# VatsalSy/gerris-fft-particles

Measured on AMD Instinct MI355X. Metric: Mcell-steps/s (projection+advection), 3D 256^3 uniform, higher is better.
Workload: dtype f64; 1 GPU; 3-D periodic Taylor-Green, 256^3 per GPU, default projection/advection parameters (SURVEY 8d config C); relax_mode=exact, parallelism=1 box, rccl_world_size=0

## Files before the change

gerris-fft-particles_amd/csrc/domain.hip:

```cpp
#include "gfship_internal.hpp"

namespace gfship {

static thread_local char g_error[1024] = "";

void set_error (const char * fmt, ...)
{
  va_list ap;
  va_start (ap, fmt);
  vsnprintf (g_error, sizeof (g_error), fmt, ap);
  va_end (ap);
}

int hip_fail (hipError_t e, const char * what, const char * file, int line)
{
  set_error ("HIP error %d (%s) in %s at %s:%d", (int) e, hipGetErrorString (e), what, file, line);
  return e == hipErrorOutOfMemory ? GFSHIP_ENOMEM : GFSHIP_EHIP;
}

Field * get_field (gfship_domain * dom, gfship_field f)
{
  if (!dom || f < 0 || (size_t) f >= dom->fields.size () || !dom->fields[f].used) {
    set_error ("invalid field handle %d", f);
    return nullptr;
// ... 132 lines not shown
  return GFSHIP_OK;
}

int gfship_domain_set_exchange (gfship_domain * dom, gfship_exchange_fn fn, void * ctx)
{
  GFSHIP_CHECK (dom != nullptr, GFSHIP_EINVAL, "null domain");
  dom->exchange = fn;
  dom->exchange_ctx = ctx;
  return GFSHIP_OK;
}

int gfship_domain_set_reduce (gfship_domain * dom, gfship_reduce_fn fn, void * ctx)
{
  GFSHIP_CHECK (dom != nullptr, GFSHIP_EINVAL, "null domain");
  dom->reduce = fn;
  dom->reduce_ctx = ctx;
  return GFSHIP_OK;
}

int gfship_domain_set_gather (gfship_domain * dom, gfship_gather_fn fn, void * ctx, int rank,
			      int nboxes, const int lattice[3])
{
  GFSHIP_CHECK (dom && lattice, GFSHIP_EINVAL, "null argument");
  GFSHIP_CHECK (nboxes >= 1 && rank >= 0 && rank < nboxes &&
		(long) lattice[0]*lattice[1]*lattice[2] == nboxes, GFSHIP_EINVAL,
		"box %d of %d on a lattice of %d x %d x %d", rank, nboxes, lattice[0], lattice[1], lattice[2]);
  for (int d = 0; d < 2*dom->dim; d++)
    GFSHIP_CHECK (lattice[d/2] == 1 || dom->side[d] == GFSHIP_SIDE_EXTERNAL, GFSHIP_EINVAL,
		  "side %d faces another box of the lattice: it must be GFSHIP_SIDE_EXTERNAL", d);
  dom->gather = fn;
  dom->gather_ctx = ctx;
  dom->lat_rank = rank; dom->lat_n = nboxes;
  for (int c = 0; c < 3; c++) dom->lat_b[c] = lattice[c];
  return GFSHIP_OK;
}

int gfship_domain_path_counts (gfship_domain * dom, unsigned long long * lattice_cycles,
			       unsigned long long * fused_mpi_launches)
{
  GFSHIP_CHECK (dom != nullptr, GFSHIP_EINVAL, "null domain");
  if (lattice_cycles) *lattice_cycles = dom->n_lattice_cycles;
  if (fused_mpi_launches) *fused_mpi_launches = dom->n_fused_mpi;
  return GFSHIP_OK;
}

int gfship_domain_kernel_counts (gfship_domain * dom, unsigned long long * counts, int n)
{
  GFSHIP_CHECK (dom != nullptr && counts != nullptr && n >= 0, GFSHIP_EINVAL, "null argument");
  for (int k = 0; k < n && k < GFSHIP_KC_COUNT; k++)
    counts[k] = dom->kc[k];
  return GFSHIP_OK;
}

int gfship_domain_synchronize (gfship_domain * dom)
{
  GFSHIP_CHECK (dom != nullptr, GFSHIP_EINVAL, "null domain");
  GFSHIP_HIP (hipStreamSynchronize (dom->stream));
  return GFSHIP_OK;
}

void * gfship_domain_stream (gfship_domain * dom)
{
  return dom ? (void *) dom->stream : nullptr;
}

gfship_field gfship_field_alloc (gfship_domain * dom, int component)
{
  GFSHIP_CHECK (dom != nullptr, GFSHIP_EINVAL, "null domain");
  GFSHIP_CHECK (component >= -1 && component < dom->dim, GFSHIP_EINVAL,
		"component %d out of range", component);
  size_t slot = dom->fields.size ();
  for (size_t f = 0; f < dom->fields.size (); f++)
    if (!dom->fields[f].used) { slot = f; break; }
  if (slot == dom->fields.size ())
    dom->fields.emplace_back ();
  Field nf;
  nf.used = true;
  nf.component = component;
  size_t total = 0;
  for (int l = 0; l <= dom->depth; l++)
    total += (dom->lay[l].total + 31) & ~(size_t) 31;
  double * base = nullptr;
  GFSHIP_HIP (hipMalloc ((void **) &base, total*sizeof (double)));
  GFSHIP_HIP (hipMemsetAsync (base, 0, total*sizeof (double), dom->stream));
  size_t o = 0;
  for (int l = dom->depth; l >= 0; l--) {
    nf.lev[l] = base + o;
    nf.zero[l] = true;
    o += (dom->lay[l].total + 31) & ~(size_t) 31;
  }
  dom->fields[slot] = nf;
  return (gfship_field) slot;
}

int gfship_field_free (gfship_domain * dom, gfship_field f)
{
  Field * F = get_field (dom, f);
  if (!F) return GFSHIP_EINVAL;
  GFSHIP_HIP (hipStreamSynchronize (dom->stream));
  GFSHIP_HIP (hipFree (F->lev[dom->depth]));
  for (int d = 0; d < 6; d++)
    if (F->bcval[d]) GFSHIP_HIP (hipFree (F->bcval[d]));
  *F = Field ();
  return GFSHIP_OK;
}

// ... 131 lines not shown
```

gerris-fft-particles_amd/csrc/gfship_internal.hpp:

```cpp
#pragma once

#include <hip/hip_runtime.h>
#include <cstdio>
#include <cstdarg>
#include <cstring>
#include <vector>
#include <deque>
#include <string>
#include <type_traits>
#include "gfship.h"
#include "switches.hpp"
#include "cell_update.hpp"

namespace gfship {

struct Layout {
  int n = 0;
  int px = 0;
  int xo = 1;
  int rows = 0;
  int dim = 3;
  long sy = 0;
  long sz = 0;
  size_t total = 0;
// ... 38 lines not shown
struct RelaxOp {
  int kind = 0;
  double w = 1., h2 = 1.;
  const double * wf[6] = {};
};

inline W6 op_weights (const RelaxOp * op)
{
  W6 wf;
  for (int d = 0; d < 6; d++) wf.p[d] = op ? op->wf[d] : nullptr;
  return wf;
}

struct BcDesc {
  int side[6];
  int type[6];
  const double * val[6];
  int component;
  int homogeneous;
};

}

struct gfship_domain {
  int dim = 3, depth = 0, device = 0;
  int side[6] = {1, 1, 1, 1, 1, 1};
  int relax_mode = GFSHIP_RELAX_EXACT;
  gfship::Switches sw;
  gfship::Layout lay[GFSHIP_MAXLEVEL + 1];
  std::deque<gfship::Field> fields;
  hipStream_t stream = nullptr;
  hipEvent_t ev0 = nullptr, ev1 = nullptr;
  hipStream_t side_stream = nullptr;
  hipEvent_t side_fork = nullptr;
  int (* before_write) (void *) = nullptr;
  void * before_write_ctx = nullptr;
  double * d_scratch = nullptr;
  size_t scratch_doubles = 0;
  double * h_pinned = nullptr;
  gfship_exchange_fn exchange = nullptr; void * exchange_ctx = nullptr;
  gfship_reduce_fn reduce = nullptr;     void * reduce_ctx = nullptr;
  bool has_external = false;
  void * comm = nullptr;
  int overlap = 0;
  int lat_rank = -1, lat_n = 0, lat_b[3] = { 1, 1, 1 };
  gfship_gather_fn gather = nullptr; void * gather_ctx = nullptr;
  double * lat_res = nullptr, * lat_xch = nullptr;
  unsigned * lat_bar = nullptr;
  size_t lat_res_doubles = 0, lat_xch_doubles = 0;
  double * gfv_send[6] = {}, * gfv_recv[6] = {};
  double src[3] = { 0., 0., 0. };
  unsigned long long n_lattice_cycles = 0, n_fused_mpi = 0;
  unsigned long long kc[GFSHIP_KC_COUNT] = {};
  bool lattice_attr_set = false;
  void * mpi_plan[GFSHIP_MAXLEVEL + 1] = {};
  gfship_field dp_cache = -1;
  int skew_resident = -1;
  int patch_resident = 0;
  bool no_fused_godunov = false;
  bool no_fused_loop = false;
  bool force_hyperplane = false;
  bool unit_weights = false;
  bool weighted = false;
  unsigned long weights_stamp = 0;
  gfship_field wf[6] = {-1, -1, -1, -1, -1, -1};
  gfship::SkewPlan skew[GFSHIP_MAXLEVEL + 1];
  double diff_w[GFSHIP_MAXLEVEL + 1] = {};
  double * cfl_partial = nullptr;
  size_t cfl_nblocks = 0, cfl_used = 0;
  bool cfl_dirty = false;
  bool coarse_attr_set = false;
  gfship_field res_cache = -1;
  bool diff_ready = false;
  int diff_kind = 1;
  int patch_call = -1;
};

namespace gfship {

void set_error (const char * fmt, ...);
int  hip_fail (hipError_t e, const char * what, const char * file, int line);

inline int before_write (gfship_domain * dom)
{
  return dom->before_write ? dom->before_write (dom->before_write_ctx) : GFSHIP_OK;
}

#define GFSHIP_HIP(call) do { hipError_t e_ = (call); \
    if (e_ != hipSuccess) return gfship::hip_fail (e_, #call, __FILE__, __LINE__); } while (0)

inline hipError_t stream_wait_spin (hipStream_t st)
{
  hipError_t e;
  while ((e = hipStreamQuery (st)) == hipErrorNotReady)
    ;
  return e;
}

template <class F> inline void with_bools (F && f) { f (); }
template <class F, class... B> inline void with_bools (F && f, bool b0, B... rest)
{
  if (b0) with_bools ([&] (auto... r) { f (std::true_type {}, r...); }, rest...);
  else    with_bools ([&] (auto... r) { f (std::false_type {}, r...); }, rest...);
}

template <class F, class... B> inline void with_kind (F && f, int kind, B... bools)
// ... 182 lines not shown
```

gerris-fft-particles_amd/csrc/poisson_kernels.hip:

```cpp
#include "gfship_internal.hpp"
#include "cell_loop.hpp"
#include "relax_skew.hpp"
#include <algorithm>
#include <cstdlib>

namespace gfship {

template <int DIM, int OP>
__device__ __forceinline__ double relax_value (const double * __restrict__ u, long c, long sy, long sz,
					       double rhs, double dia, unsigned dimension,
					       double omega, double w, double h2, const W6 * wf = nullptr)
{
  return cell_update<DIM, OP> (kind_weights<OP> (w, ArrayW { wf, c }), ArrayU { u, c, sy, sz }, rhs, dia, u + c,
			       dimension, omega, h2);
}

__device__ __forceinline__ double relax_value_six (const double * __restrict__ u, long c, long sy, long sz,
						    double rhs)
{
  return cell_update_six (ArrayU { u, c, sy, sz }, rhs);
}

template <int DIM, int OP>
__global__ void __launch_bounds__(256)
// ... 1003 lines not shown
  return GFSHIP_OK;
}

template <int DIM>
__global__ void __launch_bounds__(256)
relax_redblack_kernel (Layout L, int colour, unsigned dimension, double omega,
		       double * __restrict__ u, const double * __restrict__ rhs,
		       const double * __restrict__ dia)
{
  int n = L.n;
  int half = (n + 1)/2;
  int ih = blockIdx.x*blockDim.x + threadIdx.x;
  int j = blockIdx.y + 1;
  int k = DIM == 3 ? blockIdx.z + 1 : 0;
  if (ih >= half) return;
  int i = 2*ih + 1 + ((j + k + colour) & 1);
  if (i > n) return;
  long c = L.idx (i, j, k);
  u[c] = relax_value<DIM, 0> (u, c, L.sy, L.sz, rhs[c], dia[c], dimension, omega, 1., 1.);
}

int launch_relax_redblack (gfship_domain * dom, unsigned dimension, int level, double omega,
			   double * u, const double * rhs, const double * dia)
{
  const Layout & L = dom->lay[level];
  int half = (L.n + 1)/2;
  int block = half >= 128 ? 128 : 64;
  dim3 grid ((half + block - 1)/block, L.n, dom->dim == 3 ? L.n : 1);
  for (int colour = 0; colour < 2; colour++) {
    with_bools ([&] (auto D3) {
      hipLaunchKernelGGL (relax_redblack_kernel<decltype (D3)::value ? 3 : 2>, grid, dim3 (block), 0, dom->stream,
			  L, colour, dimension, omega, u, rhs, dia);
    }, dom->dim == 3);
  }
  GFSHIP_HIP (hipGetLastError ());
  return GFSHIP_OK;
}

template <int DIM>
__global__ void __launch_bounds__(256)
residual_kernel (Layout L, const double * __restrict__ u, const double * __restrict__ rhs,
		 const double * __restrict__ dia, double * __restrict__ res)
{
  CELL_LOOP_PROLOGUE (L);
  const FaceSums s = face_sums<DIM> (UnitW {}, ArrayU { u, c, L.sy, L.sz }, dia[c]);
  res[c] = residual_close (s.a, s.b, rhs[c], u[c]);
}

template <bool NORM>
__global__ void residual_norm2_kernel (Layout L, const double * __restrict__ u, const double * __restrict__ rhs,
				       const double * __restrict__ dia, double * __restrict__ res, double inv,
				       double weight, double * __restrict__ partial);

int launch_residual (gfship_domain * dom, int level, const double * u, const double * rhs,
		     const double * dia, double * res)
{
  const Layout & L = dom->lay[level];
  dim3 grid, block;
  cell_grid (L, &grid, &block);
  const bool pairs = dom->sw.residual_pairs;
  if (dom->dim == 3 && L.n >= 64) dom->kc[pairs ? GFSHIP_KC_RESIDUAL_PAIRS : GFSHIP_KC_RESIDUAL_SCALAR]++;
  if (dom->dim == 3 && L.n >= 64 && pairs) {
    const long nitems = (long) L.n*L.n*(L.n/2);
    long nb = (nitems + 255)/256;
    if (nb > 4096) nb = 4096;
    hipLaunchKernelGGL (residual_norm2_kernel<false>, dim3 ((int) nb), dim3 (256), 0, dom->stream, L, u, rhs,
			dia, res, 1., 1., nullptr);
    GFSHIP_HIP (hipGetLastError ());
    return GFSHIP_OK;
  }
  with_bools ([&] (auto D3) {
    hipLaunchKernelGGL (residual_kernel<decltype (D3)::value ? 3 : 2>, grid, block, 0, dom->stream, L, u, rhs, dia, res);
  }, dom->dim == 3);
  GFSHIP_HIP (hipGetLastError ());
  return GFSHIP_OK;
}

template <int DIM>
__global__ void __launch_bounds__(256)
residual_weighted_kernel (Layout L, const double * __restrict__ u, const double * __restrict__ rhs,
			  const double * __restrict__ dia, double * __restrict__ res, W6 wf)
{
  CELL_LOOP_PROLOGUE (L);
  const FaceSums s = face_sums<DIM> (ArrayW { &wf, c }, ArrayU { u, c, L.sy, L.sz }, dia[c]);
  res[c] = residual_close (s.a, s.b, rhs[c], u[c]);
}

RelaxOp weighted_op (gfship_domain * dom, int level)
{
  RelaxOp op;
  op.kind = 2;
  for (int d = 0; d < 2*dom->dim; d++)
    op.wf[d] = dom->fields[dom->wf[d]].lev[level];
  return op;
}

int launch_residual_weighted (gfship_domain * dom, int level, const double * u, const double * rhs,
			      const double * dia, double * res)
{
  const Layout & L = dom->lay[level];
  dim3 grid, block;
  cell_grid (L, &grid, &block);
  RelaxOp op = weighted_op (dom, level);
  W6 wf = op_weights (&op);
  with_bools ([&] (auto D3) {
    hipLaunchKernelGGL (residual_weighted_kernel<decltype (D3)::value ? 3 : 2>, grid, block, 0, dom->stream, L, u, rhs,
			dia, res, wf);
  }, dom->dim == 3);
  GFSHIP_HIP (hipGetLastError ());
  return GFSHIP_OK;
}

struct A3 { const double * p[3]; };
struct M6 { double * p[6]; };

// ... 386 lines not shown
    if (dia) di = *(const d2 *) (dia + c);
    d2 out;
    {
      double a = di.x, b = 0.;
      a += 1.; b += 1.*uc.y;
      a += 1.; b += 1.*ul;
      a += 1.; b += 1.*ut.x;
      a += 1.; b += 1.*ub.x;
      a += 1.; b += 1.*uf.x;
      a += 1.; b += 1.*uk.x;
      out.x = rh.x - (b - uc.x*a);
    }
    {
      double a = di.y, b = 0.;
      a += 1.; b += 1.*ur;
      a += 1.; b += 1.*uc.x;
      a += 1.; b += 1.*ut.y;
      a += 1.; b += 1.*ub.y;
      a += 1.; b += 1.*uf.y;
      a += 1.; b += 1.*uk.y;
      out.y = rh.y - (b - uc.y*a);
    }
    *(d2 *) (res + c) = out;
    if (NORM)
#pragma unroll
    for (int e = 0; e < 2; e++) {
      const double raw = e ? out.y : out.x;
      double val = raw*inv;
      s0 += weight*val;
      val = fabs (val);
      s3 = fmax (s3, val);
      s1 += weight*val;
      s2 += weight*val*val;
      s4 += raw;
    }
  }
  if (!NORM) return;
  __shared__ double sh[5][4];
  s0 = wave_sum (s0); s1 = wave_sum (s1); s2 = wave_sum (s2); s3 = wave_max (s3); s4 = wave_sum (s4);
  int w = threadIdx.x >> 6, lane = threadIdx.x & 63;
  if (lane == 0) { sh[0][w] = s0; sh[1][w] = s1; sh[2][w] = s2; sh[3][w] = s3; sh[4][w] = s4; }
  __syncthreads ();
  if (threadIdx.x == 0) {
    int nw = blockDim.x >> 6;
    double r0 = 0., r1 = 0., r2 = 0., r3 = 0., r4 = 0.;
    for (int q = 0; q < nw; q++) {
      r0 += sh[0][q]; r1 += sh[1][q]; r2 += sh[2][q]; r3 = fmax (r3, sh[3][q]); r4 += sh[4][q];
    }
    double * p = partial + 5*(size_t) blockIdx.x;
    p[0] = r0; p[1] = r1; p[2] = r2; p[3] = r3; p[4] = r4;
  }
}

int launch_residual_norm (gfship_domain * dom, int level, const double * u, const double * rhs,
			  const double * dia, double * res, double scale, double weight,
			  double * out, bool dia_zero)
{
  const Layout & L = dom->lay[level];
  if (!power_of_two (scale)) {
    int r = launch_residual (dom, level, u, rhs, dia, res);
    if (r) return r;
    return out ? launch_norm (dom, level, res, scale, weight, out) :
      launch_norm_async (dom, level, res, scale, weight);
  }
  long nrows = L.dim == 3 ? (long) L.n*L.n : L.n;
  int block = L.n >= 256 ? 256 : L.n >= 128 ? 128 : 64;
  int rn_blocks = dom->sw.rn_blocks;
  if (rn_blocks < 64 || rn_blocks > 8192) rn_blocks = 4096;
  int nblocks = (int) (nrows > rn_blocks ? rn_blocks : nrows);
  double * partial = dom->d_scratch;
  double * result = out ? dom->h_pinned : dom->h_pinned + 8;
  const bool rn_pairs = dom->sw.residual_pairs;
  if (dom->dim == 3 && L.n >= 64) dom->kc[rn_pairs ? GFSHIP_KC_RESIDUAL_PAIRS : GFSHIP_KC_RESIDUAL_SCALAR]++;
  if (dom->dim == 3 && L.n >= 64 && rn_pairs) {
    const long nitems = (long) L.n*L.n*(L.n/2);
    long nb = (nitems + 255)/256;
    nblocks = (int) (nb > rn_blocks ? rn_blocks : nb);
    hipLaunchKernelGGL (residual_norm2_kernel<true>, dim3 (nblocks), dim3 (256), 0, dom->stream, L, u,
			rhs, dia_zero ? nullptr : dia, res, 1./scale, weight, partial);
  }
  else
    with_bools ([&] (auto D3) {
      hipLaunchKernelGGL (residual_norm_kernel<decltype (D3)::value ? 3 : 2>, dim3 (nblocks), dim3 (block), 0,
			  dom->stream, L, u, rhs, dia_zero ? nullptr : dia, res, 1./scale, weight, partial);
    }, dom->dim == 3);
  hipLaunchKernelGGL (norm_final_kernel, dim3 (1), dim3 (256), 0, dom->stream,
		      partial, nblocks, result);
  GFSHIP_HIP (hipGetLastError ());
  dom->kc[GFSHIP_KC_RN_BLOCKS_LIMIT] = rn_blocks;
  if ((unsigned long long) nblocks > dom->kc[GFSHIP_KC_RN_BLOCKS_MAX])
    dom->kc[GFSHIP_KC_RN_BLOCKS_MAX] = nblocks;
  if (out) {
    GFSHIP_HIP (stream_wait_spin (dom->stream));
    memcpy (out, dom->h_pinned, 5*sizeof (double));
  }
  return GFSHIP_OK;
}

struct MpiOrderPlan {
  int * cells = nullptr;
  std::vector<int> first;
  int shell_steps = 0;
};

template <int DIM, int OP>
__global__ void __launch_bounds__(256)
relax_listed_kernel (const int * __restrict__ cells, int count, long sy, long sz,
		     unsigned dimension, double omega, double w, double h2,
		     double * __restrict__ u, const double * __restrict__ rhs,
		     const double * __restrict__ dia)
{
  const int q = blockIdx.x*blockDim.x + threadIdx.x;
  if (q >= count) return;
  const long c = cells[q];
  u[c] = relax_value<DIM, OP> (u, c, sy, sz, rhs[c], dia[c], dimension, omega, w, h2);
}

static inline unsigned long long morton_key (int dim, int level, int I, int J, int K)
{
  unsigned long long m = 0;
  for (int b = level - 1; b >= 0; b--) {
    unsigned n = ((I >> b) & 1) | (((J >> b) & 1) << 1) | (dim == 3 ? ((K >> b) & 1) << 2 : 0);
    m = (m << (dim == 3 ? 3 : 2)) | n;
  }
  return m;
}

// ... 126 lines not shown
```

gerris-fft-particles_amd/gfship/__init__.py:

```python
import ctypes as C
import os
import sys

import numpy as np

_PKG = os.path.dirname(os.path.dirname(os.path.abspath(__file__)))
LIB_PATH = os.environ.get("GFSHIP_LIB", os.path.join(_PKG, "lib", "libgfship.so"))

SIDE_PERIODIC, SIDE_BOUNDARY, SIDE_EXTERNAL = 0, 1, 2
BC_SYMMETRY, BC_DIRICHLET, BC_NEUMANN = 0, 1, 2
SCHEME_GODUNOV, SCHEME_NONE = 0, 1
RELAX_EXACT, RELAX_REDBLACK, RELAX_EXACT_HYPERPLANE, RELAX_EXACT_PER_SWEEP = 0, 1, 2, 3


class GfshipError(RuntimeError):
    pass


class Norm(C.Structure):
    _fields_ = [("bias", C.c_double), ("first", C.c_double), ("second", C.c_double),
                ("infty", C.c_double), ("w", C.c_double)]


class MultilevelParams(C.Structure):
# ... 47 lines not shown
    "gfship_diffusion_rhs": (_i, [_vp, _i, _i, _i, _d]),
    "gfship_diffusion_residual": (_i, [_vp, _i, _i, _i, _i]),
    "gfship_diffusion_cycle": (_i, [_vp, _u, _u, _u, _i, _i, _i, _i]),
    "gfship_diffusion": (_i, [_vp, C.POINTER(MultilevelParams), _i, _i, _i]),
    "gfship_time_relax": (_i, [_vp, _u, _i, _i, _i, _i, _i, _pd]),
    "gfship_time_relax_loop": (_i, [_vp, _i, _i, _i, _i, _u, _i, _pd, _pi]),
    "gfship_time_relax_loop_inclusive": (_i, [_vp, _i, _i, _i, _i, _u, _i, _pd, _pi, _pd]),
    "gfship_sim_create": (_i, [C.POINTER(_vp), _vp]),
    "gfship_sim_destroy": (None, [_vp]),
    "gfship_sim_variable": (_i, [_vp, _i, _i]),
    "gfship_sim_projection_params": (C.POINTER(MultilevelParams), [_vp]),
    "gfship_sim_approx_projection_params": (C.POINTER(MultilevelParams), [_vp]),
    "gfship_sim_advection_params": (C.POINTER(AdvectionParams), [_vp]),
    "gfship_sim_set_time": (_i, [_vp, _d, _d]),
    "gfship_sim_set_next_event": (_i, [_vp, _vp, _vp]),
    "gfship_sim_time": (_d, [_vp]),
    "gfship_sim_iter": (_u, [_vp]),
    "gfship_sim_add_tracer": (_i, [_vp]),
    "gfship_sim_set_viscosity": (_i, [_vp, _i, _d]),
    "gfship_sim_set_viscosity_faces": (_i, [_vp, _i, _pi]),
    "gfship_sim_set_alpha_cell": (_i, [_vp, _i]),
    "gfship_sim_set_viscosity_cell": (_i, [_vp, _i]),
    "gfship_variable_mac_source": (_i, [_vp, _i, _i]),
    "gfship_sim_set_alpha": (_i, [_vp, _pi]),
    "gfship_sim_set_source": (_i, [_vp, _i, _d]),
    "gfship_sim_diffusion_params": (C.POINTER(MultilevelParams), [_vp, _i]),
    "gfship_sim_start": (_i, [_vp]),
    "gfship_sim_step": (_i, [_vp]),
    "gfship_sim_advection_step": (_i, [_vp]),
    "gfship_sim_set_tracer_gradient": (_i, [_vp, _i, _i]),
    "gfship_sim_set_tracer_scheme": (_i, [_vp, _i, _i]),
    "gfship_sim_set_tracer_diffusion": (_i, [_vp, _i, _d]),
    "gfship_sim_tracer_diffusion_params": (C.POINTER(MultilevelParams), [_vp, _i]),
    "gfship_sim_tracer_diffusion_path": (_i, [_vp, _i]),
    "gfship_sim_tracer_diffusion_counts": (_i, [_vp, C.POINTER(C.c_ulonglong)]),
    "gfship_predicted_face_velocities": (_i, [_vp]),
    "gfship_mac_projection": (_i, [_vp, C.POINTER(MultilevelParams), _d, _i, _pi]),
    "gfship_approximate_projection": (_i, [_vp, C.POINTER(MultilevelParams), _d, _i, _pi]),
    "gfship_centered_velocity_advection": (_i, [_vp, _pi, _pi]),
    "gfship_correct_centered_velocities": (_i, [_vp, _pi, _d]),
    "gfship_sim_advance_time": (_i, [_vp]),
    "gfship_tracer_advection": (_i, [_vp, _i, _d]),
    "gfship_domain_cfl": (_i, [_vp, _pd]),
    "gfship_set_timestep": (_i, [_vp]),
    "gfship_coarse_init": (_i, [_vp]),
    "gfship_divergence_norm": (_i, [_vp, C.POINTER(Norm)]),
    "gfship_sim_download_un": (_i, [_vp, _i, _pd]),
    "gfship_domain_set_overlap": (_i, [_vp, _i]),
    "gfship_domain_set_exchange": (_i, [_vp, _vp, _vp]),
    "gfship_domain_set_reduce": (_i, [_vp, _vp, _vp]),
    "gfship_domain_set_gather": (_i, [_vp, _vp, _vp, _i, _i, C.POINTER(C.c_int)]),
    "gfship_domain_path_counts": (_i, [_vp, C.POINTER(C.c_ulonglong), C.POINTER(C.c_ulonglong)]),
    "gfship_domain_kernel_counts": (_i, [_vp, C.POINTER(C.c_ulonglong), _i]),
    "gfship_sim_restart": (_i, [_vp, _d, _u]),
    "gfship_snapshot_tree_bytes": (C.c_size_t, [_vp, _i]),
    "gfship_snapshot_tree_write": (_i, [_vp, _i, _pi, _vp, C.c_size_t]),
    "gfship_snapshot_tree_read": (_i, [_vp, _i, _pi, _vp, C.c_size_t]),
    "gfship_comm_available": (_i, []),
    "gfship_comm_unique_id": (_i, [_vp]),
    "gfship_domain_comm_init": (_i, [_vp, _vp, _i, _i, _pi]),
    "gfship_domain_comm_size": (_i, [_vp]),
    "gfship_domain_comm_stats": (_i, [_vp, C.POINTER(C.c_ulonglong), C.POINTER(C.c_ulonglong)]),
    "gfship_domain_comm_destroy": (_i, [_vp]),
    "gfship_halo_pack": (_i, [_vp, _vp, _i, _i, _vp]),
    "gfship_halo_unpack": (_i, [_vp, _vp, _i, _i, _vp]),
    "gfship_halo_pack_sides": (_i, [_vp, _vp, _i, _i, _pi, C.POINTER(_vp)]),
    "gfship_halo_unpack_sides": (_i, [_vp, _vp, _i, _i, _pi, C.POINTER(_vp)]),
    "gfship_field_interpolate": (_i, [_vp, _i, _i, _pd, _pd, C.POINTER(C.c_ubyte)]),
    "gfship_particles_create": (_i, [C.POINTER(_vp), _vp, _i, _pd, C.POINTER(C.c_uint)]),
    "gfship_particles_destroy": (None, [_vp]),
    "gfship_particle_list_event": (_i, [_vp]),
    "gfship_particles_count": (_i, [_vp]),
    "gfship_particles_set_migrate": (_i, [_vp, _vp, _vp]),
    "gfship_particles_slots": (_i, [_vp]),
    "gfship_particles_record_size": (_i, [_vp]),
    "gfship_particles_sort": (_i, [_vp]),
    "gfship_particles_set_sort_interval": (_i, [_vp, _i]),
    "gfship_particles_download": (_i, [_vp, _pd, C.POINTER(C.c_uint)]),
    "gfship_particles_download_old": (_i, [_vp, _pd]),
    "gfship_energy_spectra_bins": (_i, [_vp]),
    "gfship_energy_spectra": (_i, [_vp, _i, C.POINTER(_i), _pd, C.POINTER(C.c_double),
                                   C.POINTER(C.c_double)]),
    "gfship_init_spectra": (_i, [_vp, _vp, C.POINTER(_i)]),
    "gfship_output_spectra_side": (_i, [_vp]),
    "gfship_output_spectra": (_i, [_vp, _i, _pd, C.POINTER(C.c_double)]),
    "gfship_output_spectra_plane": (_i, [_vp, _i, _i, _d, _pd, _pd]),
    "gfship_turbulent_viscosity": (_i, [_vp, C.POINTER(_i), C.c_double, _i, _i]),
    "gfship_particles_set_particulate": (_i, [_vp, _pd, _pd, _pd]),
    "gfship_particles_set_forces": (_i, [_vp, _i, C.POINTER(_i), _pd]),
    "gfship_particles_set_force_coefficient": (_i, [_vp, _i, C.c_char_p]),
    "gfship_particles_download_particulate": (_i, [_vp, _pd, _pd, _pd]),
    "gfship_particulate_field": (_i, [_vp, _i]),
    "gfship_particles_forces_on_fluid": (_i, [_vp]),
    "gfship_particles_set_kernel": (_i, [_vp, C.c_double, C.c_char_p]),
    "gfship_source_particulate_event": (_i, [_vp, C.POINTER(_i)]),
    "gfship_particles_spread_forces": (_i, [_vp, C.POINTER(_i)]),
    "gfship_sim_set_source_fields": (_i, [_vp, C.POINTER(_i)]),
    "gfship_particles_time_spreading": (_i, [_vp, C.POINTER(_i), _pd]),
    "gfship_tree_create": (_i, [C.POINTER(_vp), _i, C.c_void_p, _vp, _i]),
    "gfship_tree_create_sides": (_i, [C.POINTER(_vp), _i, C.c_void_p, _vp, _pi, _i]),
    "gfship_tree_set_bc": (_i, [_vp, _i, _i]),
    "gfship_tree_poisson_solve": (_i, [_vp, C.POINTER(MultilevelParams), _d]),
    "gfship_tree_destroy": (None, [_vp]),
    "gfship_tree_depth": (_i, [_vp]),
    "gfship_tree_dim": (_i, [_vp]),
    "gfship_tree_flags": (_i, [_vp, _i, C.POINTER(C.c_ubyte)]),
    "gfship_tree_upload": (_i, [_vp, _i, _i, _pd]),
    "gfship_tree_download": (_i, [_vp, _i, _i, _pd]),
    "gfship_tree_projection_params": (C.POINTER(MultilevelParams), [_vp, _i]),
    "gfship_tree_set_time": (_i, [_vp, _d, _d]),
    "gfship_tree_set_next_event": (_i, [_vp, _vp, _vp]),
    "gfship_tree_time": (_d, [_vp]),
    "gfship_tree_dt": (_d, [_vp]),
    "gfship_tree_iter": (_u, [_vp]),
    "gfship_tree_add_tracer": (_i, [_vp, _i]),
    "gfship_tree_set_bc_u": (_i, [_vp, _i, _i, _i]),
    "gfship_tree_set_viscosity": (_i, [_vp, _i, _d]),
    "gfship_tree_set_source": (_i, [_vp, _i, _d]),
    "gfship_tree_diffusion_params": (C.POINTER(MultilevelParams), [_vp, _i]),
    "gfship_tree_start": (_i, [_vp]),
    "gfship_tree_step": (_i, [_vp]),
    "gfship_tree_snapshot_bytes": (C.c_size_t, [_vp, _i]),
    "gfship_tree_snapshot_write": (_i, [_vp, _i, _pi, _vp, C.c_size_t]),
    "gfship_tree_snapshot_read": (_i, [_vp, _i, _pi, _vp, C.c_size_t]),
    "gfship_tree_restart": (_i, [_vp, _d, _u]),
    "gfship_tree_sweep_levels": (_i, [_vp, _i, _pi, _pi]),
    "gfship_tree_divergence": (_i, [_vp]),
    "gfship_tree_host_check": (_i, [_i, C.c_void_p, _vp, _pi, _u, C.POINTER(C.c_longlong)]),
    "gfship_tree_host_check_diffusion": (_i, [_i, C.c_void_p, _vp, _pi, _u, _d, C.POINTER(C.c_longlong)]),
}


UNIQUE_ID_BYTES = 128

KERNEL_COUNT_NAMES = (
    "PREDICT_SWEEP", "PREDICT_SWEEP_MPI", "PREDICT_TILED", "PREDICT_TILED_MPI", "PREDICT_GENERAL",
    "ADVECT3_SWEEP2", "ADVECT3_SWEEP2_MPI", "ADVECT3_SWEEP1", "ADVECT3_TILED", "ADVECT3_TILED_MPI",
    "ADVECT1_TILED_VELOCITY", "ADVECT1_TILED_TRACER", "ADVECT_GENERAL", "CORRECTION_FUSED",
    "CORRECTION_DECLINED", "DIVERGENCE_FUSED", "DIVERGENCE_DECLINED", "DIVERGENCE_SEPARATE",
    "PROJECT_PAIRS", "PROJECT_SCALAR", "RESIDUAL_PAIRS", "RESIDUAL_SCALAR", "RN_BLOCKS_LIMIT",
    "RN_BLOCKS_MAX", "ROWS2D", "HYPERPLANES_2D", "DIFFUSION_PIPELINED", "DIFFUSION_HYPERPLANES",
    "WEIGHTED_PIPELINED", "WEIGHTED_HYPERPLANES", "PROLONGATION_FUSED", "PROLONGATION_DECLINED",
    "RESTRICTION_FUSED", "RESTRICTION_DECLINED", "PROLONG_PACK_NEW", "PROLONG_PACK_OLD",
    "ARM_AHEAD", "ARM_AHEAD_DECLINED", "ARM_INLINE", "PATCH_LOOP_KERNEL_ARMS",
    "PATCH_LOOP_HOST_ARMS", "XCD_SCOPE_ON", "XCD_SCOPE_OFF", "XCD_NEAR_MODE", "XCD_PLACE_ON",
    "XCD_PLACE_OFF", "COARSE_CYCLES", "COARSE_THREADS", "COARSE_END_BY_LEVEL",
    "DIFFUSION_FACES_PIPELINED", "DIFFUSION_FACES_HYPERPLANES",
)
KERNEL_COUNT_VALUES = ("RN_BLOCKS_LIMIT", "RN_BLOCKS_MAX", "XCD_NEAR_MODE", "COARSE_THREADS")


def comm_available():
    _check(lib().gfship_comm_available())


def comm_unique_id():
    buf = C.create_string_buffer(UNIQUE_ID_BYTES)
    _check(lib().gfship_comm_unique_id(buf))
    return buf.raw


def lib():
    global _lib
    if _lib is None:
        if not os.path.exists(LIB_PATH):
            raise GfshipError("%s not found: run __graft_entry__.build() "
                              "(gerris-fft-particles_amd/csrc/build.sh)" % LIB_PATH)
        if "torch" not in sys.modules and os.environ.get("GFSHIP_NO_TORCH") is None:
            try:
                import torch
            except ImportError:
                pass
        L = C.CDLL(LIB_PATH)
        for name, (res, args) in SIGNATURES.items():
            f = getattr(L, name)
            f.restype, f.argtypes = res, args
        _lib = L
    return _lib


def _check(rc):
    if rc < 0:
        raise GfshipError("gfship error %d: %s" % (rc, lib().gfship_last_error().decode()))
    return rc


class Variable:

    def __init__(self, dom, component=-1):
        self.dom = dom
        self.h = _check(lib().gfship_field_alloc(dom.ptr, component))

    def _shape(self, level):
        return ((1 << level) + 2,) * self.dom.dim

    def upload(self, a, level=None):
        level = self.dom.depth if level is None else level
        a = np.ascontiguousarray(a, dtype=np.float64)
        assert a.shape == self._shape(level), (a.shape, self._shape(level))
        _check(lib().gfship_field_upload(self.dom.ptr, self.h, level, a.ctypes.data_as(_pd)))

    def download(self, level=None):
# ... 10 lines not shown
        if val is not None:
            val = np.ascontiguousarray(val, dtype=np.float64).ravel()
            p = val.ctypes.data_as(_pd)
        else:
            p = None
        _check(lib().gfship_field_set_bc(self.dom.ptr, self.h, d, kind, p))

    def free(self):
        if self.h is not None and self.dom.ptr:
            lib().gfship_field_free(self.dom.ptr, self.h)
            self.h = None


class Domain:

    def __init__(self, dim, depth, side=None, device=0):
        self.dim, self.depth = dim, depth
        s = (C.c_int * 6)(*(side if side is not None else [SIDE_BOUNDARY] * 6))
        p = _vp()
        _check(lib().gfship_domain_create(C.byref(p), dim, depth, s, device))
        self.ptr = p

    def variable(self, component=-1):
        return Variable(self, component)

    def params(self):
        par = MultilevelParams()
        lib().gfship_multilevel_params_init(C.byref(par), self.dim)
        return par

    def comm_init(self, unique_id, rank, nranks, lattice):
        buf = C.create_string_buffer(bytes(unique_id), UNIQUE_ID_BYTES)
        _check(lib().gfship_domain_comm_init(self.ptr, buf, rank, nranks, (C.c_int * 3)(*lattice)))

    def comm_size(self):
        return _check(lib().gfship_domain_comm_size(self.ptr))

    def comm_stats(self):
        m, b = C.c_ulonglong(), C.c_ulonglong()
        _check(lib().gfship_domain_comm_stats(self.ptr, C.byref(m), C.byref(b)))
        return int(m.value), int(b.value)

    def path_counts(self):
        a, b = C.c_ulonglong(), C.c_ulonglong()
        _check(lib().gfship_domain_path_counts(self.ptr, C.byref(a), C.byref(b)))
        return int(a.value), int(b.value)

    def kernel_counts(self):
        n = len(KERNEL_COUNT_NAMES)
        a = (C.c_ulonglong * n)()
        _check(lib().gfship_domain_kernel_counts(self.ptr, a, n))
        return {name: int(a[k]) for k, name in enumerate(KERNEL_COUNT_NAMES)}

    def snapshot_tree(self, variables):
        n = len(variables)
        h = (C.c_int * n)(*[v.h for v in variables])
        size = lib().gfship_snapshot_tree_bytes(self.ptr, n)
        buf = C.create_string_buffer(size)
        _check(lib().gfship_snapshot_tree_write(self.ptr, n, h, buf, size))
        return buf.raw

    def snapshot_tree_read(self, variables, data):
        n = len(variables)
        h = (C.c_int * n)(*[v.h for v in variables])
        buf = C.create_string_buffer(bytes(data), len(data))
        _check(lib().gfship_snapshot_tree_read(self.ptr, n, h, buf, len(data)))

    def set_overlap(self, overlap):
        _check(lib().gfship_domain_set_overlap(self.ptr, int(overlap)))

    def set_relax_mode(self, mode):
        _check(lib().gfship_domain_set_relax_mode(self.ptr, mode))

    def synchronize(self):
        _check(lib().gfship_domain_synchronize(self.ptr))

    def bc(self, v, v1=None, level=None):
        level = self.depth if level is None else level
        _check(lib().gfship_bc(self.ptr, v.h, (v1 or v).h, level))

    def homogeneous_bc(self, ov, v, level=None):
        level = self.depth if level is None else level
        _check(lib().gfship_homogeneous_bc(self.ptr, ov.h, v.h, level))

    def poisson_coefficients(self):
        _check(lib().gfship_poisson_coefficients(self.ptr))

    def poisson_coefficients_alpha(self, alpha):
        h = (C.c_int * 3)(*([v.h for v in alpha] + [-1] * (3 - len(alpha))))
        _check(lib().gfship_poisson_coefficients_alpha(self.ptr, h))

    def poisson_weight(self, d, level=None):
        w = C.c_int()
        _check(lib().gfship_poisson_weights(self.ptr, d, C.byref(w)))
        v = Variable.__new__(Variable)
        v.dom, v.h = self, w.value
        a = v.download(level)
        v.h = None
        return a

    def relax(self, u, rhs, dia, level=None, omega=1., d=None):
        level = self.depth if level is None else level
        _check(lib().gfship_relax(self.ptr, d or self.dim, level, omega, u.h, rhs.h, dia.h))

    def residual(self, u, rhs, dia, res, level=None, d=None):
        level = self.depth if level is None else level
# ... 560 lines not shown
```

include/gfship.h:

```cpp
#ifndef GFSHIP_H
#define GFSHIP_H

#include <stddef.h>

#ifdef __cplusplus
extern "C" {
#endif

#define GFSHIP_VERSION   1
#define GFSHIP_MAXLEVEL  12

enum { GFSHIP_OK = 0, GFSHIP_EINVAL = -1, GFSHIP_ENODEVICE = -2, GFSHIP_ENOMEM = -3,
       GFSHIP_EHIP = -4, GFSHIP_EUNSUPPORTED = -5 };

enum { GFSHIP_SIDE_PERIODIC = 0,
       GFSHIP_SIDE_BOUNDARY = 1,
       GFSHIP_SIDE_EXTERNAL = 2 };

enum { GFSHIP_BC_SYMMETRY = 0, GFSHIP_BC_DIRICHLET = 1, GFSHIP_BC_NEUMANN = 2 };

enum { GFSHIP_RELAX_EXACT = 0, GFSHIP_RELAX_REDBLACK = 1, GFSHIP_RELAX_EXACT_HYPERPLANE = 2,
       GFSHIP_RELAX_EXACT_PER_SWEEP = 3 };

typedef struct gfship_domain gfship_domain;
// ... 217 lines not shown
  GFSHIP_KC_PREDICT_SWEEP_MPI,
  GFSHIP_KC_PREDICT_TILED,
  GFSHIP_KC_PREDICT_TILED_MPI,
  GFSHIP_KC_PREDICT_GENERAL,
  GFSHIP_KC_ADVECT3_SWEEP2,
  GFSHIP_KC_ADVECT3_SWEEP2_MPI,
  GFSHIP_KC_ADVECT3_SWEEP1,
  GFSHIP_KC_ADVECT3_TILED,
  GFSHIP_KC_ADVECT3_TILED_MPI,
  GFSHIP_KC_ADVECT1_TILED_VELOCITY,
  GFSHIP_KC_ADVECT1_TILED_TRACER,
  GFSHIP_KC_ADVECT_GENERAL,
  GFSHIP_KC_CORRECTION_FUSED,
  GFSHIP_KC_CORRECTION_DECLINED,
  GFSHIP_KC_DIVERGENCE_FUSED,
  GFSHIP_KC_DIVERGENCE_DECLINED,
  GFSHIP_KC_DIVERGENCE_SEPARATE,
  GFSHIP_KC_PROJECT_PAIRS,
  GFSHIP_KC_PROJECT_SCALAR,
  GFSHIP_KC_RESIDUAL_PAIRS,
  GFSHIP_KC_RESIDUAL_SCALAR,
  GFSHIP_KC_RN_BLOCKS_LIMIT,
  GFSHIP_KC_RN_BLOCKS_MAX,
  GFSHIP_KC_ROWS2D,
  GFSHIP_KC_HYPERPLANES_2D,
  GFSHIP_KC_DIFFUSION_PIPELINED,
  GFSHIP_KC_DIFFUSION_HYPERPLANES,
  GFSHIP_KC_WEIGHTED_PIPELINED,
  GFSHIP_KC_WEIGHTED_HYPERPLANES,
  GFSHIP_KC_PROLONGATION_FUSED,
  GFSHIP_KC_PROLONGATION_DECLINED,
  GFSHIP_KC_RESTRICTION_FUSED,
  GFSHIP_KC_RESTRICTION_DECLINED,
  GFSHIP_KC_PROLONG_PACK_NEW,
  GFSHIP_KC_PROLONG_PACK_OLD,
  GFSHIP_KC_ARM_AHEAD,
  GFSHIP_KC_ARM_AHEAD_DECLINED,
  GFSHIP_KC_ARM_INLINE,
  GFSHIP_KC_PATCH_LOOP_KERNEL_ARMS,
  GFSHIP_KC_PATCH_LOOP_HOST_ARMS,
  GFSHIP_KC_XCD_SCOPE_ON,
  GFSHIP_KC_XCD_SCOPE_OFF,
  GFSHIP_KC_XCD_NEAR_MODE,
  GFSHIP_KC_XCD_PLACE_ON,
  GFSHIP_KC_XCD_PLACE_OFF,
  GFSHIP_KC_COARSE_CYCLES,
  GFSHIP_KC_COARSE_THREADS,
  GFSHIP_KC_COARSE_END_BY_LEVEL,
  GFSHIP_KC_DIFFUSION_FACES_PIPELINED,
  GFSHIP_KC_DIFFUSION_FACES_HYPERPLANES,
  GFSHIP_KC_COUNT
};
int  gfship_domain_kernel_counts (gfship_domain * dom, unsigned long long * counts, int n);
#define GFSHIP_UNIQUE_ID_BYTES 128
int  gfship_comm_available (void);
int  gfship_comm_unique_id (void * id);
int  gfship_domain_comm_init (gfship_domain * dom, const void * unique_id, int rank, int nranks,
			      const int lattice[3]);
int  gfship_domain_comm_size (gfship_domain * dom);
int  gfship_domain_comm_stats (gfship_domain * dom, unsigned long long * messages,
			       unsigned long long * bytes);
int  gfship_domain_comm_destroy (gfship_domain * dom);

int  gfship_halo_pack (gfship_domain * dom, const void * dev_ptr, int level, int side, void * dev_buf);
int  gfship_halo_unpack (gfship_domain * dom, void * dev_ptr, int level, int side, const void * dev_buf);
int  gfship_halo_pack_sides (gfship_domain * dom, const void * dev_ptr, int level, int nsides,
			     const int * sides, void * const * dev_bufs);
int  gfship_halo_unpack_sides (gfship_domain * dom, void * dev_ptr, int level, int nsides,
			       const int * sides, void * const * dev_bufs);


typedef struct gfship_tree gfship_tree;
typedef double (* gfship_refine_fn) (double x, double y, double z, void * ctx);
enum { GFSHIP_TREE_P = 0, GFSHIP_TREE_PMAC, GFSHIP_TREE_U, GFSHIP_TREE_V, GFSHIP_TREE_GX, GFSHIP_TREE_GY,
       GFSHIP_TREE_GMACX, GFSHIP_TREE_GMACY, GFSHIP_TREE_UN0, GFSHIP_TREE_UN1, GFSHIP_TREE_UN2,
       GFSHIP_TREE_UN3, GFSHIP_TREE_W, GFSHIP_TREE_GZ, GFSHIP_TREE_GMACZ, GFSHIP_TREE_UN4,
       GFSHIP_TREE_UN5, GFSHIP_TREE_DIV, GFSHIP_TREE_BCVAL, GFSHIP_TREE_RES,
       GFSHIP_TREE_T0, GFSHIP_TREE_T1, GFSHIP_TREE_BCU, GFSHIP_TREE_BCV, GFSHIP_TREE_BCW };
int  gfship_tree_create (gfship_tree ** tree, int dim, gfship_refine_fn refine, void * ctx, int device);
int  gfship_tree_create_sides (gfship_tree ** tree, int dim, gfship_refine_fn refine, void * ctx,
			       const int * side, int device);
int  gfship_tree_set_bc (gfship_tree * tree, int d, int kind);
int  gfship_tree_poisson_solve (gfship_tree * tree, gfship_multilevel_params * par, double dt);
void gfship_tree_destroy (gfship_tree * tree);
int  gfship_tree_depth (const gfship_tree * tree);
int  gfship_tree_dim (const gfship_tree * tree);
int  gfship_tree_flags (const gfship_tree * tree, int level, unsigned char * out );
int  gfship_tree_upload (gfship_tree * tree, int var, int level, const double * in );
int  gfship_tree_download (gfship_tree * tree, int var, int level, double * out);
gfship_multilevel_params * gfship_tree_projection_params (gfship_tree * tree, int approx);
int  gfship_tree_set_time (gfship_tree * tree, double end, double cfl);
int  gfship_tree_set_next_event (gfship_tree * tree, gfship_next_event_fn fn, void * ctx);
double   gfship_tree_time (const gfship_tree * tree);
double   gfship_tree_dt (const gfship_tree * tree);
unsigned gfship_tree_iter (const gfship_tree * tree);
int  gfship_tree_add_tracer (gfship_tree * tree, int gradient);
int  gfship_tree_set_bc_u (gfship_tree * tree, int c, int d, int kind);
int  gfship_tree_set_viscosity (gfship_tree * tree, int c, double nu);
int  gfship_tree_set_source (gfship_tree * tree, int c, double g);
gfship_multilevel_params * gfship_tree_diffusion_params (gfship_tree * tree, int c);
int  gfship_tree_start (gfship_tree * tree);
int  gfship_tree_step (gfship_tree * tree);
size_t gfship_tree_snapshot_bytes (const gfship_tree * tree, int nvars);
int  gfship_tree_snapshot_write (gfship_tree * tree, int nvars, const int * vars, void * host_buf, size_t bytes);
int  gfship_tree_snapshot_read (gfship_tree * tree, int nvars, const int * vars, const void * host_buf, size_t bytes);
int  gfship_tree_restart (gfship_tree * tree, double t, unsigned i);
// ... 24 lines not shown
```

Baseline: 2836 Mcell-steps/s.

## Add z-marching residual kernel with shared-memory plane reuse for large grids

```diff
diff --git a/gerris-fft-particles_amd/csrc/domain.hip b/gerris-fft-particles_amd/csrc/domain.hip
--- a/gerris-fft-particles_amd/csrc/domain.hip
+++ b/gerris-fft-particles_amd/csrc/domain.hip
@@ -208,6 +208,23 @@
   return GFSHIP_OK;
 }
 
+int gfship_domain_kernel_counts_more (gfship_domain * dom, unsigned long long * counts, int n)
+{
+  GFSHIP_CHECK (dom != nullptr && counts != nullptr && n >= 0, GFSHIP_EINVAL, "null argument");
+  for (int k = 0; k < n && k < GFSHIP_KC_MORE_COUNT; k++)
+    counts[k] = dom->kc_more[k];
+  return GFSHIP_OK;
+}
+
+int gfship_domain_set_march_min_n (gfship_domain * dom, int n)
+{
+  GFSHIP_CHECK (n >= 64 && (n & (n - 1)) == 0, GFSHIP_EINVAL,
+		"march_min_n = %d: a power of two >= 64 is expected", n);
+  GFSHIP_CHECK (dom != nullptr, GFSHIP_EINVAL, "null domain");
+  dom->march_min_n = n;
+  return GFSHIP_OK;
+}
+
 int gfship_domain_synchronize (gfship_domain * dom)
 {
   GFSHIP_CHECK (dom != nullptr, GFSHIP_EINVAL, "null domain");
diff --git a/gerris-fft-particles_amd/csrc/gfship_internal.hpp b/gerris-fft-particles_amd/csrc/gfship_internal.hpp
--- a/gerris-fft-particles_amd/csrc/gfship_internal.hpp
+++ b/gerris-fft-particles_amd/csrc/gfship_internal.hpp
@@ -114,6 +114,8 @@
   double src[3] = { 0., 0., 0. };
   unsigned long long n_lattice_cycles = 0, n_fused_mpi = 0;
   unsigned long long kc[GFSHIP_KC_COUNT] = {};
+  unsigned long long kc_more[GFSHIP_KC_MORE_COUNT] = {};
+  int march_min_n = 256;
   bool lattice_attr_set = false;
   void * mpi_plan[GFSHIP_MAXLEVEL + 1] = {};
   gfship_field dp_cache = -1;
diff --git a/gerris-fft-particles_amd/csrc/poisson_kernels.hip b/gerris-fft-particles_amd/csrc/poisson_kernels.hip
--- a/gerris-fft-particles_amd/csrc/poisson_kernels.hip
+++ b/gerris-fft-particles_amd/csrc/poisson_kernels.hip
@@ -1079,6 +1079,9 @@
 				       const double * __restrict__ dia, double * __restrict__ res, double inv,
 				       double weight, double * __restrict__ partial);
 
+static bool launch_residual_march (gfship_domain * dom, const Layout & L, const double * u, const double * rhs,
+				   const double * dia, double * res);
+
 int launch_residual (gfship_domain * dom, int level, const double * u, const double * rhs,
 		     const double * dia, double * res)
 {
@@ -1088,6 +1091,10 @@
   const bool pairs = dom->sw.residual_pairs;
   if (dom->dim == 3 && L.n >= 64) dom->kc[pairs ? GFSHIP_KC_RESIDUAL_PAIRS : GFSHIP_KC_RESIDUAL_SCALAR]++;
   if (dom->dim == 3 && L.n >= 64 && pairs) {
+    if (launch_residual_march (dom, L, u, rhs, dia, res)) {
+      GFSHIP_HIP (hipGetLastError ());
+      return GFSHIP_OK;
+    }
     const long nitems = (long) L.n*L.n*(L.n/2);
     long nb = (nitems + 255)/256;
     if (nb > 4096) nb = 4096;
@@ -1580,6 +1587,178 @@
   }
 }
 
+constexpr int MARCH_CHUNK = 32, MARCH_WIDE_N = 256;
+#define MARCH_WIDE 128, 2, 2
+#define MARCH_NARROW 32, 8, 2
+
+template <bool NORM, int PX, int RY, int RT>
+__global__ void __launch_bounds__(PX*RY)
+residual_march_kernel (Layout L, const double * __restrict__ u, const double * __restrict__ rhs,
+		       const double * __restrict__ dia, double * __restrict__ res, double inv,
+		       double weight, double * __restrict__ partial, int chunk)
+{
+  typedef double d2 __attribute__((ext_vector_type(2)));
+  constexpr int NW = PX*RY/64;
+  static_assert (PX <= 64 ? 64 % PX == 0 : PX % 64 == 0, "a row segment is a part or a multiple of a wavefront");
+  __shared__ d2 plane[2][RY*RT][PX];
+  const int n = L.n, nxs = n/(2*PX);
+  const int p = threadIdx.x % PX, r = threadIdx.x / PX;
+  const int xs = blockIdx.x % nxs, yb = blockIdx.x / nxs;
+  const int k0 = 1 + blockIdx.y*chunk, k1 = min (k0 + chunk, n + 1);
+  long c = L.idx (1 + 2*(xs*PX + p), 1 + (yb*RY + r)*RT, k0);
+  const bool lo = r == 0, hi = r == RY - 1, halo = lo || hi;
+  const bool e0 = p % 64 == 0, e1 = p % 64 == 63 || p == PX - 1;
+  const long hoff = lo ? - L.sy : RT*L.sy;
+  d2 um[RT], uc[RT], up[RT], rh[RT], di[RT];
+  double ue[RT][2];
+  d2 uh = { 0., 0. };
+#pragma unroll
+  for (int t = 0; t < RT; t++) {
+    const long ct = c + t*L.sy;
+    um[t] = *(const d2 *) (u + ct - L.sz); uc[t] = *(const d2 *) (u + ct); up[t] = *(const d2 *) (u + ct + L.sz);
+    ue[t][0] = ue[t][1] = 0.;
+    if (e0) ue[t][0] = u[ct - 1];
+    if (e1) ue[t][1] = u[ct + 2];
+    rh[t] = *(const d2 *) (rhs + ct);
+    di[t] = d2 { 0., 0. };
+    if (dia) di[t] = *(const d2 *) (dia + ct);
+    plane[0][r*RT + t][p] = uc[t];
+  }
+  if (halo) uh = *(const d2 *) (u + c + hoff);
+  __syncthreads ();
+  double s0 = 0., s1 = 0., s2 = 0., s3 = 0., s4 = 0.;
+  int buf = 0;
+  for (int k = k0; k < k1; k++, c += L.sz, buf ^= 1) {
+    d2 un[RT], rhn[RT], din[RT], uhn = { 0., 0. };
+    double uen[RT][2];
+#pragma unroll
+    for (int t = 0; t < RT; t++) {
+      un[t] = rhn[t] = din[t] = d2 { 0., 0. };
+      uen[t][0] = uen[t][1] = 0.;
+    }
+    if (k + 1 < k1) {
+#pragma unroll
+      for (int t = 0; t < RT; t++) {
+	const long ct = c + t*L.sy + L.sz;
+	un[t] = *(const d2 *) (u + ct + L.sz);
+	if (e0) uen[t][0] = u[ct - 1];
+	if (e1) uen[t][1] = u[ct + 2];
+	rhn[t] = *(const d2 *) (rhs + ct);
+	if (dia) din[t] = *(const d2 *) (dia + ct);
+      }
+      if (halo) uhn = *(const d2 *) (u + c + L.sz + hoff);
+    }
+#pragma unroll
+    for (int t = 0; t < RT; t++)
+      plane[buf ^ 1][r*RT + t][p] = up[t];
+    d2 below = uh, above = uh;
+    if (!lo) below = plane[buf][r*RT - 1][p];
+    if (!hi) above = plane[buf][r*RT + RT][p];
+#pragma unroll
+    for (int t = 0; t < RT; t++) {
+      const d2 ub = t > 0 ? uc[t > 0 ? t - 1 : 0] : below, ut = t < RT - 1 ? uc[t < RT - 1 ? t + 1 : t] : above;
+      double ul = __shfl_up (uc[t].y, 1, 64), ur = __shfl_down (uc[t].x, 1, 64);
+      if (e0) ul = ue[t][0];
+      if (e1) ur = ue[t][1];
+      d2 out;
+      {
+	double a = di[t].x, b = 0.;
+	a += 1.; b += 1.*uc[t].y;
+	a += 1.; b += 1.*ul;
+	a += 1.; b += 1.*ut.x;
+	a += 1.; b += 1.*ub.x;
+	a += 1.; b += 1.*up[t].x;
+	a += 1.; b += 1.*um[t].x;
+	out.x = rh[t].x - (b - uc[t].x*a);
+      }
+      {
+	double a = di[t].y, b = 0.;
+	a += 1.; b += 1.*ur;
+	a += 1.; b += 1.*uc[t].x;
+	a += 1.; b += 1.*ut.y;
+	a += 1.; b += 1.*ub.y;
+	a += 1.; b += 1.*up[t].y;
+	a += 1.; b += 1.*um[t].y;
+	out.y = rh[t].y - (b - uc[t].y*a);
+      }
+      *(d2 *) (res + c + t*L.sy) = out;
+      if (NORM)
+#pragma unroll
+      for (int e = 0; e < 2; e++) {
+	const double raw = e ? out.y : out.x;
+	double val = raw*inv;
+	s0 += weight*val;
+	val = fabs (val);
+	s3 = fmax (s3, val);
+	s1 += weight*val;
+	s2 += weight*val*val;
+	s4 += raw;
+      }
+    }
+    __syncthreads ();
+#pragma unroll
+    for (int t = 0; t < RT; t++) {
+      um[t] = uc[t]; uc[t] = up[t]; up[t] = un[t]; rh[t] = rhn[t]; di[t] = din[t];
+      ue[t][0] = uen[t][0]; ue[t][1] = uen[t][1];
+    }
+    uh = uhn;
+  }
+  if (NORM) {
+    static_assert (NW <= 4, "block_norm_sums reduces at most 4 wavefronts");
+    block_norm_sums (s0, s1, s2, s3, s4, partial, blockIdx.x + (size_t) gridDim.x*blockIdx.y);
+  }
+}
+
+struct MarchPlan { dim3 grid; int chunk; bool wide; };
+
+static bool march_plan (gfship_domain * dom, const Layout & L, MarchPlan * m)
+{
+  if (dom->dim != 3 || !dom->sw.residual_pairs || dom->sw.rn_blocks != 0 || L.n < dom->march_min_n || L.n % 64)
+    return false;
+  constexpr int wide[3] = { MARCH_WIDE }, narrow[3] = { MARCH_NARROW };
+  m->wide = L.n >= MARCH_WIDE_N && L.n % (2*wide[0]) == 0;
+  const int * g = m->wide ? wide : narrow;
+  const long columns = (long) (L.n/(2*g[0]))*(L.n/(g[1]*g[2]));
+  int len = MARCH_CHUNK;
+  while (len < L.n && columns*((L.n + len - 1)/len) > 8192) len *= 2;
+  if (columns*((L.n + len - 1)/len) > 8192)
+    return false;
+  m->grid = dim3 ((unsigned) columns, (unsigned) ((L.n + len - 1)/len));
+  m->chunk = len;
+  return true;
+}
+
+template <bool NORM, int PX, int RY, int RT>
+static void march_launch_geometry (gfship_domain * dom, const MarchPlan & m, const Layout & L, const double * u,
+				   const double * rhs, const double * dia, double * res, double inv, double weight,
+				   double * partial)
+{
+  hipLaunchKernelGGL ((residual_march_kernel<NORM, PX, RY, RT>), m.grid, dim3 (PX*RY), 0, dom->stream, L, u, rhs,
+		      dia, res, inv, weight, partial, m.chunk);
+}
+
+template <bool NORM>
+static void march_launch (gfship_domain * dom, const MarchPlan & m, const Layout & L, const double * u,
+			  const double * rhs, const double * dia, double * res, double inv, double weight,
+			  double * partial)
+{
+  dom->kc_more[GFSHIP_KC_RESIDUAL_MARCH]++;
+  if (m.wide)
+    march_launch_geometry<NORM, MARCH_WIDE> (dom, m, L, u, rhs, dia, res, inv, weight, partial);
+  else
+    march_launch_geometry<NORM, MARCH_NARROW> (dom, m, L, u, rhs, dia, res, inv, weight, partial);
+}
+
+static bool launch_residual_march (gfship_domain * dom, const Layout & L, const double * u, const double * rhs,
+				   const double * dia, double * res)
+{
+  MarchPlan m;
+  if (!march_plan (dom, L, &m))
+    return false;
+  march_launch<false> (dom, m, L, u, rhs, dia, res, 1., 1., nullptr);
+  return true;
+}
+
 int launch_residual_norm (gfship_domain * dom, int level, const double * u, const double * rhs,
 			  const double * dia, double * res, double scale, double weight,
 			  double * out, bool dia_zero)
@@ -1600,7 +1779,12 @@
   double * result = out ? dom->h_pinned : dom->h_pinned + 8;
   const bool rn_pairs = dom->sw.residual_pairs;
   if (dom->dim == 3 && L.n >= 64) dom->kc[rn_pairs ? GFSHIP_KC_RESIDUAL_PAIRS : GFSHIP_KC_RESIDUAL_SCALAR]++;
-  if (dom->dim == 3 && L.n >= 64 && rn_pairs) {
+  MarchPlan march;
+  if (march_plan (dom, L, &march)) {
+    nblocks = (int) (march.grid.x*march.grid.y);
+    march_launch<true> (dom, march, L, u, rhs, dia_zero ? nullptr : dia, res, 1./scale, weight, partial);
+  }
+  else if (dom->dim == 3 && L.n >= 64 && rn_pairs) {
     const long nitems = (long) L.n*L.n*(L.n/2);
     long nb = (nitems + 255)/256;
     nblocks = (int) (nb > rn_blocks ? rn_blocks : nb);
diff --git a/gerris-fft-particles_amd/gfship/__init__.py b/gerris-fft-particles_amd/gfship/__init__.py
--- a/gerris-fft-particles_amd/gfship/__init__.py
+++ b/gerris-fft-particles_amd/gfship/__init__.py
@@ -123,6 +123,8 @@
     "gfship_domain_set_gather": (_i, [_vp, _vp, _vp, _i, _i, C.POINTER(C.c_int)]),
     "gfship_domain_path_counts": (_i, [_vp, C.POINTER(C.c_ulonglong), C.POINTER(C.c_ulonglong)]),
     "gfship_domain_kernel_counts": (_i, [_vp, C.POINTER(C.c_ulonglong), _i]),
+    "gfship_domain_kernel_counts_more": (_i, [_vp, C.POINTER(C.c_ulonglong), _i]),
+    "gfship_domain_set_march_min_n": (_i, [_vp, _i]),
     "gfship_sim_restart": (_i, [_vp, _d, _u]),
     "gfship_snapshot_tree_bytes": (C.c_size_t, [_vp, _i]),
     "gfship_snapshot_tree_write": (_i, [_vp, _i, _pi, _vp, C.c_size_t]),
@@ -219,6 +221,7 @@
     "DIFFUSION_FACES_PIPELINED", "DIFFUSION_FACES_HYPERPLANES",
 )
 KERNEL_COUNT_VALUES = ("RN_BLOCKS_LIMIT", "RN_BLOCKS_MAX", "XCD_NEAR_MODE", "COARSE_THREADS")
+KERNEL_COUNT_NAMES_MORE = ("RESIDUAL_MARCH",)
 
 
 def comm_available():
@@ -335,6 +338,15 @@
         _check(lib().gfship_domain_kernel_counts(self.ptr, a, n))
         return {name: int(a[k]) for k, name in enumerate(KERNEL_COUNT_NAMES)}
 
+    def kernel_counts_more(self):
+        n = len(KERNEL_COUNT_NAMES_MORE)
+        a = (C.c_ulonglong * n)()
+        _check(lib().gfship_domain_kernel_counts_more(self.ptr, a, n))
+        return {name: int(a[k]) for k, name in enumerate(KERNEL_COUNT_NAMES_MORE)}
+
+    def set_march_min_n(self, n):
+        _check(lib().gfship_domain_set_march_min_n(self.ptr, n))
+
     def snapshot_tree(self, variables):
         n = len(variables)
         h = (C.c_int * n)(*[v.h for v in variables])
diff --git a/include/gfship.h b/include/gfship.h
--- a/include/gfship.h
+++ b/include/gfship.h
@@ -293,6 +293,12 @@
   GFSHIP_KC_COUNT
 };
 int  gfship_domain_kernel_counts (gfship_domain * dom, unsigned long long * counts, int n);
+enum {
+  GFSHIP_KC_RESIDUAL_MARCH = 0,
+  GFSHIP_KC_MORE_COUNT
+};
+int  gfship_domain_kernel_counts_more (gfship_domain * dom, unsigned long long * counts, int n);
+int  gfship_domain_set_march_min_n (gfship_domain * dom, int n);
 #define GFSHIP_UNIQUE_ID_BYTES 128
 int  gfship_comm_available (void);
 int  gfship_comm_unique_id (void * id);
```

Result: no change. 2864 Mcell-steps/s, median of 6 (+1.0%).
